# nyu-systems/Grendel-GS

Measured on AMD Instinct MI355X. Metric: training iters/sec (fwd+bwd), higher is better.
Workload: dtype f32

## Files before the change

grendel-gs_amd/csrc/composite.hip:

```cpp
#include "common.h"

namespace {

constexpr float LOG2E = 1.4426950408889634f;
constexpr float ALPHA_MIN = 1.0f / 255.0f;
constexpr float T_STOP = 0.0001f;

__device__ unsigned long long g_walked[2];

#ifdef GSR_STATS
__device__ unsigned long long g_stats[8];
#define GSR_STAT(i, v) do { const unsigned long long sv__ = (unsigned long long)(v); if (lane == 0) atomicAdd(&g_stats[i], sv__); } while (0)
#else
#define GSR_STAT(i, v) do { } while (0)
#endif

struct Entry {
    float x, y;
    float a2, b2, c2;
    float o;
    bool relevant;
};

#ifndef GSR_NO_LOG2O
#define GSR_LOG2O 1
#endif
__device__ __forceinline__ float entry_exponent(const float4 q0, const float4 q1, float dx, float dy) {
#ifdef GSR_LOG2O
    return fmaf(fmaf(q0.z, dx, q0.w * dy), dx, fmaf(q1.x * dy, dy, q1.y));
#else
    return (q0.z * dx + q0.w * dy) * dx + q1.x * dy * dy;
#endif
}
__device__ __forceinline__ float entry_alpha_raw(const float4 q1, float pe) {
#ifdef GSR_LOG2O
    return __builtin_amdgcn_exp2f(pe);
#else
    return q1.y * __builtin_amdgcn_exp2f(pe);
#endif
}
__device__ __forceinline__ bool entry_power_ok(const float4 q1, float pe) {
#ifdef GSR_LOG2O
    return pe <= q1.y;
#else
    return pe <= 0.f;
#endif
}

__device__ __forceinline__ float entry_opacity_term(float o) {
#ifdef GSR_LOG2O
    return __log2f(o);
#else
    return o;
#endif
}

__device__ __forceinline__ Entry load_entry(bool have, uint32_t id, const float2 *__restrict__ means2D,
                                            const float4 *__restrict__ conic_opacity, float qx0, float qy0) {
    Entry e;
    e.x = e.y = e.a2 = e.b2 = e.c2 = e.o = 0.f;
    e.relevant = false;
    if (have) {
        const float2 xy = means2D[id];
        const float4 co = conic_opacity[id];
        e.x = xy.x;
        e.y = xy.y;
        e.a2 = -0.5f * LOG2E * co.x;
        e.b2 = -LOG2E * co.y;
        e.c2 = -0.5f * LOG2E * co.z;
        e.o = entry_opacity_term(co.w);
        e.relevant = gsr_can_touch_box(xy, co, qx0, qy0, qx0 + 7.0f, qy0 + 7.0f);
    }
    return e;
}


typedef float v2f __attribute__((ext_vector_type(2)));
constexpr int PREC = 20;
struct PairRec {
    v2f x, y, a2, b2, c2, o, r, g, b;
};
__device__ __forceinline__ void pair_store(float *__restrict__ slab, int pos, const Entry &e, float r, float g, float b) {
    float *rec = slab + (pos >> 1) * PREC + (pos & 1);
    rec[0] = e.x;  rec[2] = e.y;  rec[4] = e.a2;  rec[6] = e.b2;  rec[8] = e.c2;
    rec[10] = e.o; rec[12] = r;   rec[14] = g;    rec[16] = b;
}
__device__ __forceinline__ PairRec pair_load(const float *__restrict__ slab, int pair) {
    const float4 *q = reinterpret_cast<const float4 *>(slab + pair * PREC);
    const float4 q0 = q[0], q1 = q[1], q2 = q[2], q3 = q[3];
    const float2 q4 = *reinterpret_cast<const float2 *>(q + 4);
    PairRec p;
    p.x = v2f{q0.x, q0.y};  p.y = v2f{q0.z, q0.w};  p.a2 = v2f{q1.x, q1.y};  p.b2 = v2f{q1.z, q1.w};
    p.c2 = v2f{q2.x, q2.y}; p.o = v2f{q2.z, q2.w};  p.r = v2f{q3.x, q3.y};   p.g = v2f{q3.z, q3.w};
    p.b = v2f{q4.x, q4.y};
    return p;
}
__device__ __forceinline__ v2f pair_exponent(const PairRec &p, float pxf, float pyf) {
    const v2f dx = p.x - pxf, dy = p.y - pyf;
    return __builtin_elementwise_fma(__builtin_elementwise_fma(p.a2, dx, p.b2 * dy), dx,
                                     __builtin_elementwise_fma(p.c2 * dy, dy, p.o));
}

__device__ __forceinline__ int composite_tile_of_block(const int2 *__restrict__ ranges, int gx, int tiles) {
    const int2 hull = ranges[tiles];
    const int gy = tiles / gx;
    if (hull.x < 0 || hull.y > gy || hull.x >= hull.y) return gsr_xcd_span_of_block(blockIdx.x, tiles);
    return gsr_xcd_span_of_block_band(blockIdx.x, tiles, hull.x * gx, (hull.y - hull.x) * gx);
}

struct RawEntry {
    float2 xy;
    float4 co;
    float r, g, b;
};
__device__ __forceinline__ RawEntry load_raw(bool have, uint32_t id, const float2 *__restrict__ means2D,
                                             const float4 *__restrict__ conic_opacity, const float *__restrict__ rgb) {
    RawEntry e;
    e.xy = make_float2(0.f, 0.f);
    e.co = make_float4(0.f, 0.f, 0.f, 0.f);
    e.r = e.g = e.b = 0.f;
    if (have) {
        e.xy = means2D[id];
        e.co = conic_opacity[id];
        e.r = rgb[3 * (size_t)id];
        e.g = rgb[3 * (size_t)id + 1];
        e.b = rgb[3 * (size_t)id + 2];
    }
    return e;
}

#ifndef GSR_SEG_LEN
#define GSR_SEG_LEN 256
#endif
#ifndef GSR_SEG_MAXJ
#define GSR_SEG_MAXJ 16
#endif
constexpr int SEG_LEN = GSR_SEG_LEN;
constexpr int SEG_MAXJ = GSR_SEG_MAXJ;
static_assert(SEG_LEN % 64 == 0 && (SEG_LEN & (SEG_LEN - 1)) == 0 && SEG_MAXJ <= 31,
              "segment geometry: K8 finds boundaries with c & (SEG_LEN - 1), so SEG_LEN is a power of two");
constexpr int SEG_WORKERS = 1024;
constexpr int SEG_SLOT_FLOATS = 7 * 256;
struct SegWs {
    uint32_t *hdr;
    uint32_t *queue;
    int32_t *seg_slot;
    float *ckpt;
    uint32_t cap;
};
__host__ __device__ inline size_t seg_ws_bytes(int tiles, uint32_t cap) {
    return 64 + sizeof(uint32_t) * (size_t)cap + sizeof(int32_t) * (size_t)tiles * SEG_MAXJ + sizeof(float) * SEG_SLOT_FLOATS * (size_t)cap;
}
inline SegWs seg_ws_of(void *ws, int tiles, uint32_t cap) {
    SegWs w{};
    if (!ws) return w;
    char *b = reinterpret_cast<char *>(ws);
    w.hdr = reinterpret_cast<uint32_t *>(b);
    w.queue = reinterpret_cast<uint32_t *>(b + 64);
    w.seg_slot = reinterpret_cast<int32_t *>(b + 64 + sizeof(uint32_t) * (size_t)cap);
    w.ckpt = reinterpret_cast<float *>(b + 64 + sizeof(uint32_t) * (size_t)cap + sizeof(int32_t) * (size_t)tiles * SEG_MAXJ);
    w.cap = cap;
    return w;
}
constexpr uint32_t SEG_CAP = 8192;

__device__ __forceinline__ int k8_checkpoint(const SegWs &seg, int *s_slot, int tile, int c, int lane,
                                                       int wave, float T, float c0, float c1, float c2) {
    const int j = c / SEG_LEN - 1;
    int slot = 0;
    if (lane == 0) {
        int v = atomicCAS(&s_slot[j], -1, -2);
        if (v == -1) {
            const uint32_t k = atomicAdd(seg.hdr, 1u);
            v = k < seg.cap ? (int)k : -3;
            if (v >= 0) {
                seg.queue[k] = (uint32_t)tile * 32u + (uint32_t)(j + 1);
                seg.seg_slot[(size_t)tile * SEG_MAXJ + j] = v;
            }
            __hip_atomic_store(&s_slot[j], v, __ATOMIC_RELEASE, __HIP_MEMORY_SCOPE_WORKGROUP);
        } else {
            while (v == -2) v = __hip_atomic_load(&s_slot[j], __ATOMIC_ACQUIRE, __HIP_MEMORY_SCOPE_WORKGROUP);
        }
        slot = v;
    }
    slot = __builtin_amdgcn_readfirstlane(slot);
    if (slot >= 0) {
        float *ck = seg.ckpt + (size_t)slot * SEG_SLOT_FLOATS + wave * 64 + lane;
        ck[0] = T;
        ck[256] = c0;
        ck[512] = c1;
        ck[768] = c2;
    }
    return slot;
}

template <bool SEG, bool BAND>
__global__ void __launch_bounds__(256)
composite_forward_kernel(int W, int H, int gx, const int2 *__restrict__ ranges,
                         const uint32_t *__restrict__ point_list, const float2 *__restrict__ means2D,
                         const float4 *__restrict__ conic_opacity, const float *__restrict__ rgb,
                         const uint8_t *__restrict__ compute_locally, const float *__restrict__ bg,
                         float *__restrict__ out_color, float *__restrict__ final_T, int32_t *__restrict__ n_contrib,
                         const SegWs seg, int band_first, int band_tiles, uint4 *__restrict__ zero16,
                         size_t zero16_n) {
    const size_t HW = (size_t)H * W;
    for (size_t i = (size_t)blockIdx.x * 256 + threadIdx.x; i < zero16_n; i += (size_t)gridDim.x * 256)
        zero16[i] = make_uint4(0u, 0u, 0u, 0u);
    int tile;
    bool idle = false;
    if (BAND) {
        if (band_first < 0) {
            const int gy = (H + GSR_BLOCK_Y - 1) / GSR_BLOCK_Y;
            int2 hull = ranges[gx * gy];
            if (hull.x < 0 || hull.y > gy || hull.x >= hull.y) hull = make_int2(0, 0);
            band_first = hull.x * gx;
            band_tiles = min((hull.y - hull.x) * gx, band_tiles);
            idle = (int)blockIdx.x >= band_tiles;
        }
        tile = band_first + (idle ? 0 : gsr_xcd_span_of_block(blockIdx.x, band_tiles));
    } else {
        tile = composite_tile_of_block(ranges, gx, (int)gridDim.x);
    }
    auto clear_outside = [&]() {
        if (!BAND) return;
        const size_t n0 = (size_t)min(H, (band_first / gx) * GSR_BLOCK_Y) * W;
        const size_t p1 = (size_t)min(H, ((band_first + band_tiles) / gx) * GSR_BLOCK_Y) * W;
        const size_t nout = n0 + (HW - p1);
        for (size_t i = (size_t)blockIdx.x * 256 + threadIdx.x; i < nout; i += (size_t)gridDim.x * 256) {
            const size_t q = i < n0 ? i : p1 + (i - n0);
            out_color[q] = 0.f;
            out_color[HW + q] = 0.f;
            out_color[2 * HW + q] = 0.f;
            final_T[q] = 1.f;
            n_contrib[q] = 0;
        }
    };
    if (idle) {
        clear_outside();
        return;
    }
    const int lane = threadIdx.x & 63, wave = threadIdx.x >> 6;
    const int tx = tile % gx, ty = tile / gx;
    const int qx0 = tx * GSR_BLOCK_X + (wave & 1) * 8, qy0 = ty * GSR_BLOCK_Y + (wave >> 1) * 8;
    const int px = qx0 + (lane & 7), py = qy0 + (lane >> 3);
    const bool inside = px < W && py < H;
    const size_t pid = (size_t)py * W + px;

    if (!compute_locally[tile]) {
        if (inside) {
            out_color[pid] = 0.f;
            out_color[HW + pid] = 0.f;
            out_color[2 * HW + pid] = 0.f;
            final_T[pid] = 1.f;
            n_contrib[pid] = 0;
        }
        clear_outside();
        return;
    }
    const int2 range = ranges[tile];
    const int n = range.y - range.x;
    const float pxf = (float)px, pyf = (float)py;

    float T = 1.0f, C0 = 0.f, C1 = 0.f, C2 = 0.f;
    int last = 0;
    bool done = !inside;
    __shared__ __attribute__((aligned(16))) float slab[4][32 * PREC];
    __shared__ int s_walk[2];
    __shared__ int s_slot[SEG_MAXJ];
    if (threadIdx.x < 2) s_walk[threadIdx.x] = 0;
    if (SEG && threadIdx.x < SEG_MAXJ) {
        s_slot[threadIdx.x] = -1;
        if (seg.seg_slot) seg.seg_slot[(size_t)tile * SEG_MAXJ + threadIdx.x] = -1;
    }
    __syncthreads();
    v2f A0 = {0.f, 0.f}, A1 = {0.f, 0.f}, A2 = {0.f, 0.f};
    v2f B0 = {0.f, 0.f}, B1 = {0.f, 0.f}, B2 = {0.f, 0.f};
    int nstored = 0;
    float *wslab = slab[wave];
    int walked = 0;

    for (int c = 0; c < n; c += 64) {
        if (__all(done)) break;
        if (SEG && seg.seg_slot && c > 0 && (c & (SEG_LEN - 1)) == 0 && c <= SEG_LEN * SEG_MAXJ) {
            if (k8_checkpoint(seg, s_slot, tile, c, lane, wave, T, B0.x + B0.y, B1.x + B1.y, B2.x + B2.y) >= 0) {
                B0 = B1 = B2 = v2f{0.f, 0.f};
                nstored = c / SEG_LEN;
            }
        }
        walked = c + 64;
        const bool have = c + lane < n;
        const uint32_t id = have ? point_list[range.x + c + lane] : 0u;
        const Entry e = load_entry(have, id, means2D, conic_opacity, (float)qx0, (float)qy0);
        float r = 0.f, g = 0.f, b = 0.f;
        if (e.relevant) {
            r = rgb[3 * (size_t)id];
            g = rgb[3 * (size_t)id + 1];
            b = rgb[3 * (size_t)id + 2];
        }
        unsigned long long m = __ballot(e.relevant);
        GSR_STAT(0, __popcll(__ballot(have)));
        GSR_STAT(1, __popcll(m));
        const int nrel = __popcll(m);
        if (e.relevant) pair_store(wslab, __popcll(m & ((1ull << lane) - 1ull)), e, r, g, b);
        {
            const int pad = (-nrel) & 3, slot = nrel + lane / 9;
            if (lane < 9 * pad) wslab[(slot >> 1) * PREC + 2 * (lane % 9) + (slot & 1)] = 0.f;
        }
        for (int p0 = 0; p0 < nrel; p0 += 4) {
            float al[4];
            bool ok[4];
            int kk[4];
            v2f cr[2], cg[2], cb[2];
#pragma unroll
            for (int h = 0; h < 2; h++) {
                const PairRec pr = pair_load(wslab, (p0 >> 1) + h);
                const v2f pe = pair_exponent(pr, pxf, pyf);
                cr[h] = pr.r;
                cg[h] = pr.g;
                cb[h] = pr.b;
#pragma unroll
                for (int u = 0; u < 2; u++) {
                    const bool live = m != 0;
                    kk[2 * h + u] = live ? __builtin_ctzll(m) : 0;
                    m &= m - 1;
                    const float pe1 = u ? pe.y : pe.x, lo = u ? pr.o.y : pr.o.x;
                    al[2 * h + u] = fminf(0.99f, __builtin_amdgcn_exp2f(pe1));
                    ok[2 * h + u] = live && pe1 <= lo && al[2 * h + u] >= ALPHA_MIN;
                }
            }
            float wv[4];
#pragma unroll
            for (int u = 0; u < 4; u++) {
                const bool take = !done && ok[u];
                const float w0 = al[u] * T;
                const float test_T = T - w0;
                const bool stop = take && __float_as_int(test_T) < __float_as_int(T_STOP);
                done = done || stop;
                const bool blend = take && !stop;
                wv[u] = blend ? w0 : 0.f;
                T = blend ? test_T : T;
                last = blend ? c + kk[u] + 1 : last;
            }
#pragma unroll
            for (int h = 0; h < 2; h++) {
                const v2f w2 = {wv[2 * h], wv[2 * h + 1]};
                A0 = __builtin_elementwise_fma(cr[h], w2, A0);
                A1 = __builtin_elementwise_fma(cg[h], w2, A1);
                A2 = __builtin_elementwise_fma(cb[h], w2, A2);
                if (SEG) {
                    B0 = __builtin_elementwise_fma(cr[h], w2, B0);
                    B1 = __builtin_elementwise_fma(cg[h], w2, B1);
                    B2 = __builtin_elementwise_fma(cb[h], w2, B2);
                }
            }
            if (__all(done)) break;
        }
    }
    if (lane == 0) {
        atomicMax(&s_walk[0], walked < n ? walked : n);
        if (atomicAdd(&s_walk[1], 1) == 3) atomicAdd(&g_walked[0], (unsigned long long)s_walk[0]);
    }
    C0 = A0.x + A0.y;
    C1 = A1.x + A1.y;
    C2 = A2.x + A2.y;
    if (SEG && nstored > 0) {
        float r0 = B0.x + B0.y, r1 = B1.x + B1.y, r2 = B2.x + B2.y;
        for (int j = nstored - 1; j >= 0; j--) {
            float *ck = seg.ckpt + (size_t)s_slot[j] * SEG_SLOT_FLOATS + wave * 64 + lane;
            ck[1024] = r0;
            ck[1280] = r1;
            ck[1536] = r2;
            r0 += ck[256];
            r1 += ck[512];
            r2 += ck[768];
        }
    }
    if (inside) {
        out_color[pid] = C0 + T * bg[0];
        out_color[HW + pid] = C1 + T * bg[1];
        out_color[2 * HW + pid] = C2 + T * bg[2];
        final_T[pid] = T;
        n_contrib[pid] = last;
    }
    clear_outside();
}

typedef float f32x4 __attribute__((ext_vector_type(4)));

constexpr int MB = 8;
constexpr int MSTR = 66;

__device__ __forceinline__ void
composite_backward_segment(const int tile, const int sidx, int W, int H, int gx, const int2 *__restrict__ ranges,
                           const uint32_t *__restrict__ point_list, const float2 *__restrict__ means2D,
                           const float4 *__restrict__ conic_opacity, const float *__restrict__ rgb,
                           const uint8_t *__restrict__ compute_locally, const float *__restrict__ bg,
                           const float *__restrict__ final_T, const int32_t *__restrict__ n_contrib,
                           const float *__restrict__ dL_dpixels, double *__restrict__ dL_record,
                           const SegWs &seg, uint8_t *__restrict__ touched) {
    if (!compute_locally[tile]) return;
    const int lane = threadIdx.x & 63, wave = threadIdx.x >> 6;
    const int tx = tile % gx, ty = tile / gx;
    const int qx0 = tx * GSR_BLOCK_X + (wave & 1) * 8, qy0 = ty * GSR_BLOCK_Y + (wave >> 1) * 8;
    const int px = qx0 + (lane & 7), py = qy0 + (lane >> 3);
    const bool inside = px < W && py < H;
    const size_t pid = (size_t)py * W + px;
    const size_t HW = (size_t)H * W;
    const int2 range = ranges[tile];
    const float pxf = (float)px, pyf = (float)py;

    const int c_lo = sidx * SEG_LEN;
    int end_slot = -1;
    if (seg.seg_slot && sidx < SEG_MAXJ) end_slot = seg.seg_slot[(size_t)tile * SEG_MAXJ + sidx];
    const int c_hi = end_slot >= 0 ? c_lo + SEG_LEN : 0x7fffffff;
    const float T_final = inside ? final_T[pid] : 0.f;
    const int last = inside ? n_contrib[pid] : 0;
    float g0 = 0.f, g1 = 0.f, g2 = 0.f;
    if (inside) {
        g0 = dL_dpixels[pid];
        g1 = dL_dpixels[HW + pid];
        g2 = dL_dpixels[2 * HW + pid];
    }
    const float tb = T_final * (bg[0] * g0 + bg[1] * g1 + bg[2] * g2);
    const float ddelx_dx = 0.5f * W, ddely_dy = 0.5f * H;

    __shared__ float2 smat[4][MB * MSTR];
    __shared__ float sacc[4][64 * 9];
    __shared__ __attribute__((aligned(16))) float slab[4][32 * PREC];
    __shared__ float fslab[64 * 7];
    __shared__ float sout[64 * 10];
    __shared__ int s_wmax[4];
    int wmax = min(last, c_hi);
#pragma unroll
    for (int d = 32; d >= 1; d >>= 1) wmax = max(wmax, __shfl_xor(wmax, d, 64));
    if (wmax <= c_lo) wmax = 0;
    if (lane == 0) s_wmax[wave] = wmax;
    for (int i = threadIdx.x; i < 4 * 64 * 9; i += 256) (&sacc[0][0])[i] = 0.f;
    __syncthreads();
    const int bmax = max(max(s_wmax[0], s_wmax[1]), max(s_wmax[2], s_wmax[3]));
    if (bmax == 0) return;
    if (threadIdx.x == 0) atomicAdd(&g_walked[1], (unsigned long long)(bmax - c_lo));
    int wbest = 0;
#pragma unroll
    for (int w = 1; w < 4; w++)
        if (s_wmax[w] > s_wmax[wbest]) wbest = w;

    const int kq = lane >> 4, j = lane & 15;
    float Bop[16];
    {
        const bool isg = j >= 6 && j < 9;
        const float xa = (j == 0 || j == 2 || j == 5) ? 1.f : 0.f, xb1 = (j == 1 || j == 4) ? 1.f : 0.f, xc = j == 3 ? 1.f : 0.f;
        const float ya = (j == 0 || j == 1 || j == 3) ? 1.f : 0.f, yb1 = (j == 2 || j == 4) ? 1.f : 0.f, yc = j == 5 ? 1.f : 0.f;
        const float xl = (float)((wave & 1) * 8 + kq);
        float X[2];
#pragma unroll
        for (int h = 0; h < 2; h++) {
            const float x = xl + 4.f * h;
            X[h] = fmaf(x, fmaf(xc, x, xb1), xa);
        }
        const int gx0 = qx0 + kq;
        const int cx0 = min(gx0, W - 1), cx1 = min(gx0 + 4, W - 1);
        const float *gb = dL_dpixels + (size_t)(isg ? j - 6 : 0) * HW;
        float G[16];
#pragma unroll
        for (int t = 0; t < 16; t++) G[t] = 0.f;
        if (isg) {
#pragma unroll
            for (int t = 0; t < 16; t++) G[t] = gb[(size_t)min(qy0 + (t >> 1), H - 1) * W + ((t & 1) ? cx1 : cx0)];
        }
#pragma unroll
        for (int t = 0; t < 16; t++) {
            const float y = (float)((wave >> 1) * 8 + (t >> 1));
            const float Y = fmaf(y, fmaf(yc, y, yb1), ya);
            const bool inb = ((t & 1) ? gx0 + 4 : gx0) < W && qy0 + (t >> 1) < H;
            Bop[t] = isg ? (inb ? G[t] : 0.f) : X[t & 1] * Y;
        }
    }
    const float *arow = reinterpret_cast<const float *>(&smat[wave][(j & 7) * MSTR + kq]) + (j >> 3);
    const bool my_cols = kq < 2 ? j < 6 : (j >= 6 && j < 9);
    float *wslab = slab[wave];

    float T = T_final;
    float rho = 0.f;
    if (end_slot >= 0 && last > c_hi) {
        const float *ck = seg.ckpt + (size_t)end_slot * SEG_SLOT_FLOATS + wave * 64 + lane;
        T = ck[0];
        rho = (ck[1024] * g0 + ck[1280] * g1 + ck[1536] * g2) * __builtin_amdgcn_rcpf(T);
    }

    const int c0 = ((bmax - 1) / 64) * 64;
    uint32_t id_cur = (c0 + lane < wmax) ? point_list[range.x + c0 + lane] : 0u;
    uint32_t id_nxt = (c0 >= c_lo + 64 && c0 - 64 + lane < wmax) ? point_list[range.x + c0 - 64 + lane] : 0u;
    RawEntry raw = load_raw(c0 + lane < wmax, id_cur, means2D, conic_opacity, rgb);

    for (int c = c0; c >= c_lo; c -= 64) {
        float *acc_tab = sacc[wave];
        const bool have_nxt = c >= c_lo + 64 && c - 64 + lane < wmax;
        const RawEntry raw_nxt = load_raw(have_nxt, id_nxt, means2D, conic_opacity, rgb);
        const uint32_t id_nxt2 = (c >= c_lo + 128 && c - 128 + lane < wmax) ? point_list[range.x + c - 128 + lane] : 0u;
        if (c < wmax) {
            const bool have = c + lane < wmax;
            Entry e;
            e.x = raw.xy.x;
            e.y = raw.xy.y;
            e.a2 = -0.5f * LOG2E * raw.co.x;
            e.b2 = -LOG2E * raw.co.y;
            e.c2 = -0.5f * LOG2E * raw.co.z;
            e.o = entry_opacity_term(raw.co.w);
            e.relevant = have && gsr_can_touch_box(raw.xy, raw.co, (float)qx0, (float)qy0, (float)qx0 + 7.0f, (float)qy0 + 7.0f);
            unsigned long long m = __ballot(e.relevant);
            GSR_STAT(0, __popcll(__ballot(have)));
            GSR_STAT(1, __popcll(m));
            GSR_STAT(6, 1);
            if (e.relevant) pair_store(wslab, __popcll((m >> lane) >> 1), e, raw.r, raw.g, raw.b);
            if (wave == wbest) {
                float *fe = &fslab[7 * lane];
                fe[0] = e.x;  fe[1] = e.y;  fe[2] = e.a2;  fe[3] = e.b2;  fe[4] = e.c2;
                fe[5] = __uint_as_float(id_cur);
                fe[6] = raw.co.w;
            }
            unsigned long long sk = 0ull;
            auto contract_batch = [&](int filled) {
                __builtin_amdgcn_wave_barrier();
                f32x4 acc = {0.f, 0.f, 0.f, 0.f}, acc1 = {0.f, 0.f, 0.f, 0.f};
#pragma unroll
                for (int t = 0; t < 16; t += 2) {
                    acc = __builtin_amdgcn_mfma_f32_16x16x4f32(arow[8 * t], Bop[t], acc, 0, 0, 0);
                    acc1 = __builtin_amdgcn_mfma_f32_16x16x4f32(arow[8 * t + 8], Bop[t + 1], acc1, 0, 0, 0);
                }
                acc += acc1;
                const uint32_t sk4 = (kq & 1) ? (uint32_t)(sk >> 32) : (uint32_t)sk;
#pragma unroll
                for (int r4 = 0; r4 < 4; r4++) {
                    const int slot = 4 * (kq & 1) + r4;
                    if (slot < filled && my_cols) acc_tab[(int)((sk4 >> (8 * r4)) & 0xffu) * 9 + j] = acc[r4];
                }
                GSR_STAT(5, 1);
                __builtin_amdgcn_wave_barrier();
                sk = 0ull;
            };
            int s = 0;
            for (int pi = 0; m; pi++) {
                const int ka = 63 - __builtin_clzll(m);
                m &= ~(1ull << ka);
                const bool two = m != 0ull;
                const int kb = two ? 63 - __builtin_clzll(m) : ka;
                m &= ~(1ull << kb);
                const PairRec pr = pair_load(wslab, pi);
                const v2f pe = pair_exponent(pr, pxf, pyf);
                const float aar = __builtin_amdgcn_exp2f(pe.x), bar = __builtin_amdgcn_exp2f(pe.y);
                const float aal = fminf(0.99f, aar), bal = fminf(0.99f, bar);
                const bool atake = (c + ka + 1 <= last) && pe.x <= pr.o.x && aal >= ALPHA_MIN;
                const bool btake = two && (c + kb + 1 <= last) && pe.y <= pr.o.y && bal >= ALPHA_MIN;
                const v2f cg = __builtin_elementwise_fma(pr.b, v2f{g2, g2}, __builtin_elementwise_fma(pr.g, v2f{g1, g1}, pr.r * g0));
                GSR_STAT(2, two ? 2 : 1);
                GSR_STAT(3, (__builtin_amdgcn_ballot_w64(atake) != 0ull) + (__builtin_amdgcn_ballot_w64(btake) != 0ull));
                GSR_STAT(4, __popcll(__builtin_amdgcn_ballot_w64(atake)) + __popcll(__builtin_amdgcn_ballot_w64(btake)));
                const v2f qa = {atake ? aar : 0.f, atake ? aal : 0.f};
                const v2f qb = {btake ? bar : 0.f, btake ? bal : 0.f};
                const v2f inv = {__builtin_amdgcn_rcpf(1.f - qa.y), __builtin_amdgcn_rcpf(1.f - qb.y)};
                const v2f tbi = inv * tb;
                {
                    const float Tn = T * inv.x;
                    const float dot = cg.x - rho;
                    const float da = fmaf(dot, Tn, -tbi.x);
                    const v2f qw = qa * v2f{da, Tn};
                    smat[wave][s * MSTR + lane] = make_float2(qw.x, qw.y);
                    rho = fmaf(qa.y, dot, rho);
                    T = Tn;
                }
                sk |= (unsigned long long)ka << (8 * s);
                s++;
                if (two) {
                    const float Tn = T * inv.y;
                    const float dot = cg.y - rho;
                    const float da = fmaf(dot, Tn, -tbi.y);
                    const v2f qw = qb * v2f{da, Tn};
                    smat[wave][s * MSTR + lane] = make_float2(qw.x, qw.y);
                    rho = fmaf(qb.y, dot, rho);
                    T = Tn;
                    sk |= (unsigned long long)kb << (8 * s);
                    s++;
                }
                if (s == MB) {
                    contract_batch(MB);
                    s = 0;
                }
            }
            if (s > 0) contract_batch(s);
        }
        __syncthreads();
        if (wave == ((c >> 6) & 3)) {
            const float tx0 = (float)(tx * GSR_BLOCK_X), ty0 = (float)(ty * GSR_BLOCK_Y);
            const int e9 = 9 * lane;
            float Sv[9];
#pragma unroll
            for (int v = 0; v < 9; v++) Sv[v] = (sacc[0][e9 + v] + sacc[1][e9 + v]) + (sacc[2][e9 + v] + sacc[3][e9 + v]);
            const float *fe = &fslab[7 * lane];
            const float ex = fe[0] - tx0, ey = fe[1] - ty0;
            const float cA = fe[2] * (-2.0f / LOG2E), cB = fe[3] * (-1.0f / LOG2E), cC = fe[4] * (-2.0f / LOG2E);
            const float A0 = Sv[0], Ax = Sv[1], Ay = Sv[2];
            const float Mx = fmaf(ex, A0, -Ax), My = fmaf(ey, A0, -Ay);
            float o[9];
            o[0] = -(cA * Mx + cB * My) * ddelx_dx;
            o[1] = -(cB * Mx + cC * My) * ddely_dy;
            o[2] = Sv[6];
            o[3] = Sv[7];
            o[4] = Sv[8];
            o[5] = -0.5f * (fmaf(fmaf(ex, A0, -2.f * Ax), ex, Sv[3]));
            o[6] = -(fmaf(ex, My, -ey * Ax) + Sv[4]);
            o[7] = -0.5f * (fmaf(fmaf(ey, A0, -2.f * Ay), ey, Sv[5]));
            o[8] = A0 == 0.f ? 0.f : A0 / fe[6];
            const bool live = c + lane < bmax;
            float *so = &sout[10 * lane];
#pragma unroll
            for (int v = 0; v < 9; v++) so[v] = live ? o[v] : 0.f;
            so[9] = fe[5];
        }
        __syncthreads();
#pragma unroll
        for (int r = 0; r < 3; r++) {
            const int idx = threadIdx.x + 256 * r;
            const int e = idx / 9, col = idx - 9 * e;
            if (idx < 576) {
                const float val = sout[10 * e + col];
#ifndef GSR_ABL_NOATOMIC
                if (val != 0.f) {
                    const uint32_t id = __float_as_uint(sout[10 * e + 9]);
                    atomicAdd(dL_record + 9 * (size_t)id + col, (double)val);
                    if (touched) touched[id] = 1;
                }
#else
                asm volatile("" ::"v"(val));
#endif
            }
        }
#pragma unroll
        for (int i = 0; i < 9; i++) acc_tab[64 * i + lane] = 0.f;
        raw = raw_nxt;
        id_cur = id_nxt;
        id_nxt = id_nxt2;
    }
}

// ... 159 lines not shown
```

grendel-gs_amd/csrc/loss.hip:

```cpp
#include "common.h"

namespace {

__constant__ const float WIN[11] = {1.0283801239e-03f, 7.5987582095e-03f, 3.6000773311e-02f, 1.0936068743e-01f,
                                    2.1300552785e-01f, 2.6601171494e-01f, 2.1300552785e-01f, 1.0936068743e-01f,
                                    3.6000773311e-02f, 7.5987582095e-03f, 1.0283801239e-03f};
constexpr int LT = 512;
constexpr int VO = 1024 / LT;
constexpr int TW = 32, TH = 32;
constexpr int HW = TW + 10, HH = TH + 10;
constexpr int HSTR = TW + 8;
constexpr int TS = TW;
constexpr float SSIM_C1 = 0.01f * 0.01f;
constexpr float SSIM_C2 = 0.03f * 0.03f;

__device__ __forceinline__ float block_sum(float v, float *smem) {
    const int lane = threadIdx.x & 63, wave = threadIdx.x >> 6;
#pragma unroll
    for (int d = 32; d >= 1; d >>= 1) v += __shfl_xor(v, d, 64);
    if (lane == 0) smem[wave] = v;
    __syncthreads();
    float r = 0.f;
    for (int w = 0; w < LT / 64; w++) r += smem[w];
    __syncthreads();
    return r;
}

typedef float v2f __attribute__((ext_vector_type(2)));

__device__ __forceinline__ int loss_tile(int gxT, int gyT, int &c, int &ox, int &oy, int nwg) {
    const int lin = gsr_xcd_span_of_block(blockIdx.x, nwg);
    c = lin / (gxT * gyT);
    const int rem = lin - c * (gxT * gyT);
    const int by = rem / gxT;
    ox = (rem - by * gxT) * TW;
    oy = by * TH;
    return lin;
}
__device__ __forceinline__ bool loss_band(const int *__restrict__ band, int rows_cap, int W, int gxT, int &rows, int &gyT,
                                          int &nwg, long long &row_off) {
    nwg = gridDim.x;
    row_off = 0;
    if (!band) return true;
    const int channels = nwg / (gxT * gyT);
    const int y0 = band[0], y1 = band[1];
    rows = max(0, min(y1 - y0, rows_cap));
    gyT = (rows + TH - 1) / TH;
    nwg = channels * gxT * gyT;
    row_off = (long long)y0 * W;
    return (int)blockIdx.x < nwg;
}
constexpr int HV = (TW + 16) / 4;
static_assert(HH * HV <= LT, "one halo vector per thread");

__device__ __forceinline__ float expo_apply(const float *e, float x0, float x1, float x2) {
    return fmaf(e[0], x0, fmaf(e[1], x1, fmaf(e[2], x2, e[3])));
}

template <bool VEC, bool EXPO>
__global__ void __launch_bounds__(LT)
l1_ssim_forward_kernel(int rows, int W, int gxT, int gyT, const float *__restrict__ image, long long img_cstride,
                       const uint8_t *__restrict__ gt, float *__restrict__ partials, float *__restrict__ M1,
                       float *__restrict__ M2, float *__restrict__ M3, const int *__restrict__ band,
                       const float *__restrict__ expo) {
    __shared__ v2f sXY[HH][HW + 1];
    __shared__ v2f hAB[HH][HSTR];
    __shared__ v2f hCD[HH][HSTR];
    __shared__ float hE[HH][HSTR];
    __shared__ float red[LT / 64];
    int c, ox, oy, nwg;
    long long row_off;
    const int rows_cap = rows;
    if (!loss_band(band, rows_cap, W, gxT, rows, gyT, nwg, row_off)) {
        if (threadIdx.x < 2) partials[2 * (size_t)blockIdx.x + threadIdx.x] = 0.f;
        return;
    }
    const int tile_id = loss_tile(gxT, gyT, c, ox, oy, nwg);
    const int tid = threadIdx.x;
    const float *img_c = image + (long long)c * img_cstride + row_off;
    const uint8_t *gt_c = gt + (size_t)c * rows_cap * W;
    float e[4] = {0.f, 0.f, 0.f, 0.f};
    if (EXPO) {
#pragma unroll
        for (int i = 0; i < 4; i++) e[i] = expo[4 * c + i];
    }
    const float *img_0 = image + row_off;
    if (VEC) {
        if (tid < HH * HV) {
            const int ly = tid / HV, q = tid - ly * HV;
            const int gy = oy + ly - 5, gx0 = ox - 8 + 4 * q;
            float4 x = make_float4(0.f, 0.f, 0.f, 0.f);
            uchar4 y = make_uchar4(0, 0, 0, 0);
            if (gy >= 0 && gy < rows && gx0 >= 0 && gx0 < W) {
                if (EXPO) {
                    const float *p = img_0 + (size_t)gy * W + gx0;
                    const float4 x0 = *reinterpret_cast<const float4 *>(p);
                    const float4 x1 = *reinterpret_cast<const float4 *>(p + img_cstride);
                    const float4 x2 = *reinterpret_cast<const float4 *>(p + 2 * img_cstride);
                    x = make_float4(expo_apply(e, x0.x, x1.x, x2.x), expo_apply(e, x0.y, x1.y, x2.y),
                                    expo_apply(e, x0.z, x1.z, x2.z), expo_apply(e, x0.w, x1.w, x2.w));
                } else {
                    x = *reinterpret_cast<const float4 *>(img_c + (size_t)gy * W + gx0);
                }
                y = *reinterpret_cast<const uchar4 *>(gt_c + (size_t)gy * W + gx0);
            }
            const float xs[4] = {x.x, x.y, x.z, x.w};
            const float ys[4] = {(float)y.x, (float)y.y, (float)y.z, (float)y.w};
#pragma unroll
            for (int i = 0; i < 4; i++) {
                const int lx = 4 * q - 3 + i;
                if (lx >= 0 && lx < HW) sXY[ly][lx] = v2f{xs[i], ys[i] * (1.0f / 255.0f)};
            }
        }
    } else {
        for (int idx = tid; idx < HH * HW; idx += LT) {
            const int ly = idx / HW, lx = idx % HW;
            const int gy = oy + ly - 5, gx = ox + lx - 5;
            v2f v = {0.f, 0.f};
            if (gy >= 0 && gy < rows && gx >= 0 && gx < W) {
                if (EXPO) {
                    const float *p = img_0 + (size_t)gy * W + gx;
                    v.x = expo_apply(e, p[0], p[img_cstride], p[2 * img_cstride]);
                } else {
                    v.x = img_c[(size_t)gy * W + gx];
                }
                v.y = (float)gt_c[(size_t)gy * W + gx] * (1.0f / 255.0f);
            }
            sXY[ly][lx] = v;
        }
    }
    __syncthreads();
    for (int task = tid; task < HH * (TW / 4); task += LT) {
        const int r = task / (TW / 4), cx0 = (task % (TW / 4)) * 4;
        v2f xy[14], sq[14];
        float pr[14];
#pragma unroll
        for (int i = 0; i < 14; i++) {
            xy[i] = sXY[r][cx0 + i];
            sq[i] = xy[i] * xy[i];
            pr[i] = xy[i].x * xy[i].y;
        }
#pragma unroll
        for (int o = 0; o < 4; o++) {
            v2f a = {0.f, 0.f}, b = {0.f, 0.f};
            float e = 0.f;
#pragma unroll
            for (int k = 0; k < 11; k++) {
                const float w = WIN[k];
                a += xy[o + k] * w;
                b += sq[o + k] * w;
                e += pr[o + k] * w;
            }
            hAB[r][cx0 + o] = a;
            hCD[r][cx0 + o] = b;
            hE[r][cx0 + o] = e;
        }
    }
    __syncthreads();
    const int tx = tid % TW, ty0 = (tid / TW) * VO;
    v2f vab[VO], vcd[VO];
    float ve[VO];
    {
        v2f p[10 + VO], q[10 + VO];
        float t[10 + VO];
#pragma unroll
        for (int i = 0; i < 10 + VO; i++) {
            p[i] = hAB[ty0 + i][tx];
            q[i] = hCD[ty0 + i][tx];
            t[i] = hE[ty0 + i][tx];
        }
#pragma unroll
        for (int o = 0; o < VO; o++) {
            v2f a = {0.f, 0.f}, b = {0.f, 0.f};
            float e = 0.f;
#pragma unroll
            for (int k = 0; k < 11; k++) {
                const float w = WIN[k];
                a += p[o + k] * w;
                b += q[o + k] * w;
                e += t[o + k] * w;
            }
            vab[o] = a;
            vcd[o] = b;
            ve[o] = e;
        }
    }
    const int gx = ox + tx;
    float l1 = 0.f, ssim_sum = 0.f;
#pragma unroll
    for (int o = 0; o < VO; o++) {
        const int ty = ty0 + o, gy = oy + ty;
        if (gy < rows && gx < W) {
            const float mu1 = vab[o].x, mu2 = vab[o].y, e11 = vcd[o].x, e22 = vcd[o].y, e12 = ve[o];
            const v2f cxy = sXY[ty + 5][tx + 5];
            const float x = cxy.x, y = cxy.y;
            const float mu1_sq = mu1 * mu1, mu2_sq = mu2 * mu2, mu12 = mu1 * mu2;
            const float s1 = e11 - mu1_sq, s2 = e22 - mu2_sq, s12 = e12 - mu12;
            const float A = 2.f * mu12 + SSIM_C1, B = 2.f * s12 + SSIM_C2;
            const float Cd = mu1_sq + mu2_sq + SSIM_C1, Dd = s1 + s2 + SSIM_C2;
            const float inv_d = __builtin_amdgcn_rcpf(Dd);
            const float inv = __builtin_amdgcn_rcpf(Cd) * inv_d;
            const float ssim = A * B * inv;
            ssim_sum += ssim;
            l1 += fabsf(x - y);
            if (M1) {
                const size_t off = ((size_t)c * rows_cap + gy) * W + gx;
                M1[off] = 2.f * mu2 * (B - A) * inv - ssim * 2.f * mu1 * (Dd - Cd) * inv;
                M2[off] = -ssim * inv_d;
                M3[off] = 2.f * A * inv;
            }
        }
    }
    const float sl1 = block_sum(l1, red);
    const float sss = block_sum(ssim_sum, red);
    if (tid == 0) {
        partials[2 * (size_t)tile_id] = sl1;
        partials[2 * (size_t)tile_id + 1] = sss;
    }
}

template <bool VEC>
__global__ void __launch_bounds__(LT)
l1_ssim_backward_kernel(int rows, int W, int gxT, int gyT, const float *__restrict__ image, long long img_cstride,
                        const uint8_t *__restrict__ gt, const float *__restrict__ M1, const float *__restrict__ M2,
                        const float *__restrict__ M3, const float *__restrict__ grad_l1_sum,
                        const float *__restrict__ grad_ssim_sum, float scale_l1, float scale_ssim,
                        float *__restrict__ grad_image, long long grad_cstride, const int *__restrict__ band) {
    __shared__ float sM[3][HH][HW + 1];
    __shared__ float hor[3][HH][HSTR];
    int c, ox, oy, nwg;
    long long row_off;
    const int rows_cap = rows;
    if (!loss_band(band, rows_cap, W, gxT, rows, gyT, nwg, row_off)) return;
    loss_tile(gxT, gyT, c, ox, oy, nwg);
    const int tid = threadIdx.x;
    const size_t cbase = (size_t)c * rows_cap * W;
    if (VEC) {
        if (tid < HH * HV) {
            const int ly = tid / HV, q = tid - ly * HV;
            const int gy = oy + ly - 5, gx0 = ox - 8 + 4 * q;
            float4 a = make_float4(0.f, 0.f, 0.f, 0.f), b = a, d = a;
            if (gy >= 0 && gy < rows && gx0 >= 0 && gx0 < W) {
                const size_t o = cbase + (size_t)gy * W + gx0;
                a = *reinterpret_cast<const float4 *>(M1 + o);
                b = *reinterpret_cast<const float4 *>(M2 + o);
                d = *reinterpret_cast<const float4 *>(M3 + o);
            }
            const float as[4] = {a.x, a.y, a.z, a.w}, bs[4] = {b.x, b.y, b.z, b.w}, ds[4] = {d.x, d.y, d.z, d.w};
#pragma unroll
            for (int i = 0; i < 4; i++) {
                const int lx = 4 * q - 3 + i;
                if (lx >= 0 && lx < HW) {
                    sM[0][ly][lx] = as[i];
                    sM[1][ly][lx] = bs[i];
                    sM[2][ly][lx] = ds[i];
                }
            }
        }
    } else {
        for (int idx = tid; idx < HH * HW; idx += LT) {
            const int ly = idx / HW, lx = idx % HW;
            const int gy = oy + ly - 5, gx = ox + lx - 5;
            float a = 0.f, b = 0.f, d = 0.f;
            if (gy >= 0 && gy < rows && gx >= 0 && gx < W) {
                const size_t o = cbase + (size_t)gy * W + gx;
                a = M1[o];
                b = M2[o];
                d = M3[o];
            }
            sM[0][ly][lx] = a;
            sM[1][ly][lx] = b;
            sM[2][ly][lx] = d;
        }
    }
    __syncthreads();
    for (int task = tid; task < HH * (TW / 4); task += LT) {
        const int r = task / (TW / 4), cx0 = (task % (TW / 4)) * 4;
#pragma unroll
        for (int m = 0; m < 3; m++) {
            float v[14];
#pragma unroll
            for (int i = 0; i < 14; i++) v[i] = sM[m][r][cx0 + i];
#pragma unroll
            for (int o = 0; o < 4; o++) {
                float a = 0.f;
#pragma unroll
                for (int k = 0; k < 11; k++) a += WIN[k] * v[o + k];
                hor[m][r][cx0 + o] = a;
            }
        }
    }
    __syncthreads();
    const int tx = tid % TW, ty0 = (tid / TW) * VO;
    float cv[3][VO];
#pragma unroll
    for (int m = 0; m < 3; m++) {
        float v[10 + VO];
#pragma unroll
        for (int i = 0; i < 10 + VO; i++) v[i] = hor[m][ty0 + i][tx];
#pragma unroll
        for (int o = 0; o < VO; o++) {
            float a = 0.f;
#pragma unroll
            for (int k = 0; k < 11; k++) a += WIN[k] * v[o + k];
            cv[m][o] = a;
        }
    }
    const int gx = ox + tx;
    if (gx >= W) return;
    const float gl1 = grad_l1_sum[0] * scale_l1, gss = grad_ssim_sum[0] * scale_ssim;
#pragma unroll
    for (int o = 0; o < VO; o++) {
        const int gy = oy + ty0 + o;
        if (gy >= rows) break;
        const float x = image[(long long)c * img_cstride + row_off + (size_t)gy * W + gx];
        const float y = (float)gt[cbase + (size_t)gy * W + gx] * (1.0f / 255.0f);
        const float d = x - y;
        const float sgn = (d > 0.f ? 1.f : 0.f) - (d < 0.f ? 1.f : 0.f);
        grad_image[(long long)c * grad_cstride + row_off + (size_t)gy * W + gx] =
            gl1 * sgn + gss * (cv[0][o] + 2.f * x * cv[1][o] + y * cv[2][o]);
    }
}

__global__ void __launch_bounds__(256) l1_ssim_finalize_kernel(int nb, const float *__restrict__ partials, float c_l1,
                                                                float c_ssim, float bias, float inv_n,
                                                                float *__restrict__ out) {
    __shared__ double red[2][4];
    double a = 0.0, b = 0.0;
    const float2 *p2 = reinterpret_cast<const float2 *>(partials);
    for (int i0 = threadIdx.x; i0 < nb; i0 += 256 * 8) {
        float2 v[8];
#pragma unroll
        for (int u = 0; u < 8; u++) v[u] = p2[min(i0 + 256 * u, nb - 1)];
#pragma unroll
        for (int u = 0; u < 8; u++)
            if (i0 + 256 * u < nb) {
                a += (double)v[u].x;
                b += (double)v[u].y;
            }
    }
#pragma unroll
    for (int d = 32; d >= 1; d >>= 1) {
        a += __shfl_xor(a, d, 64);
        b += __shfl_xor(b, d, 64);
    }
    if ((threadIdx.x & 63) == 0) {
        red[0][threadIdx.x >> 6] = a;
        red[1][threadIdx.x >> 6] = b;
    }
    __syncthreads();
    if (threadIdx.x == 0) {
        const float s1 = (float)(red[0][0] + red[0][1] + red[0][2] + red[0][3]);
        const float s2 = (float)(red[1][0] + red[1][1] + red[1][2] + red[1][3]);
        out[0] = c_l1 * s1 + c_ssim * s2 + bias;
        out[1] = s1 * inv_n;
        out[2] = s2 * inv_n;
    }
}

template <bool VEC>
__global__ void __launch_bounds__(LT)
l1_ssim_backward_exposure_kernel(int rows, int W, int gxT, int gyT, const float *__restrict__ image, long long img_cstride,
                                 const uint8_t *__restrict__ gt, const float *__restrict__ M1,
                                 const float *__restrict__ M2, const float *__restrict__ M3,
                                 const float *__restrict__ grad_l1_sum, const float *__restrict__ grad_ssim_sum,
                                 float scale_l1, float scale_ssim, float *__restrict__ grad_image, long long grad_cstride,
                                 const int *__restrict__ band, const float *__restrict__ expo,
                                 float *__restrict__ expo_partials) {
    __shared__ float sM[3][HH][HW + 1];
    __shared__ float hor[3][HH][HSTR];
    __shared__ float red[12][LT / 64];
    int c0, ox, oy, nwg;
    long long row_off;
    const int rows_cap = rows;
    if (!loss_band(band, rows_cap, W, gxT, rows, gyT, nwg, row_off)) {
        if (threadIdx.x < 12) expo_partials[12 * (size_t)blockIdx.x + threadIdx.x] = 0.f;
        return;
    }
    const int tile_id = loss_tile(gxT, gyT, c0, ox, oy, nwg);
    const int tid = threadIdx.x, lane = tid & 63, wave = tid >> 6;
    const int tx = tid % TW, ty0 = (tid / TW) * VO;
    const int gx = ox + tx;
    const float gl1 = grad_l1_sum[0] * scale_l1, gss = grad_ssim_sum[0] * scale_ssim;
    float xin[3][VO], gout[3][VO];
    bool ok[VO];
#pragma unroll
    for (int o = 0; o < VO; o++) {
        const int gy = oy + ty0 + o;
        ok[o] = gx < W && gy < rows;
#pragma unroll
        for (int k = 0; k < 3; k++) {
            xin[k][o] = ok[o] ? image[(long long)k * img_cstride + row_off + (size_t)gy * W + gx] : 0.f;
            gout[k][o] = 0.f;
        }
    }
#pragma unroll 1
    for (int c = 0; c < 3; c++) {
        const size_t cbase = (size_t)c * rows_cap * W;
        if (VEC) {
            if (tid < HH * HV) {
                const int ly = tid / HV, q = tid - ly * HV;
                const int gy = oy + ly - 5, gx0 = ox - 8 + 4 * q;
                float4 a = make_float4(0.f, 0.f, 0.f, 0.f), b = a, d = a;
                if (gy >= 0 && gy < rows && gx0 >= 0 && gx0 < W) {
                    const size_t o = cbase + (size_t)gy * W + gx0;
                    a = *reinterpret_cast<const float4 *>(M1 + o);
                    b = *reinterpret_cast<const float4 *>(M2 + o);
                    d = *reinterpret_cast<const float4 *>(M3 + o);
                }
                const float as[4] = {a.x, a.y, a.z, a.w}, bs[4] = {b.x, b.y, b.z, b.w}, ds[4] = {d.x, d.y, d.z, d.w};
#pragma unroll
                for (int i = 0; i < 4; i++) {
                    const int lx = 4 * q - 3 + i;
                    if (lx >= 0 && lx < HW) {
                        sM[0][ly][lx] = as[i];
                        sM[1][ly][lx] = bs[i];
                        sM[2][ly][lx] = ds[i];
                    }
                }
            }
        } else {
            for (int idx = tid; idx < HH * HW; idx += LT) {
                const int ly = idx / HW, lx = idx % HW;
                const int gy = oy + ly - 5, gxh = ox + lx - 5;
                float a = 0.f, b = 0.f, d = 0.f;
                if (gy >= 0 && gy < rows && gxh >= 0 && gxh < W) {
                    const size_t o = cbase + (size_t)gy * W + gxh;
                    a = M1[o];
                    b = M2[o];
                    d = M3[o];
                }
                sM[0][ly][lx] = a;
                sM[1][ly][lx] = b;
                sM[2][ly][lx] = d;
            }
        }
        __syncthreads();
        for (int task = tid; task < HH * (TW / 4); task += LT) {
            const int r = task / (TW / 4), cx0 = (task % (TW / 4)) * 4;
#pragma unroll
            for (int m = 0; m < 3; m++) {
                float v[14];
#pragma unroll
                for (int i = 0; i < 14; i++) v[i] = sM[m][r][cx0 + i];
#pragma unroll
                for (int o = 0; o < 4; o++) {
                    float a = 0.f;
#pragma unroll
                    for (int k = 0; k < 11; k++) a = fmaf(WIN[k], v[o + k], a);
                    hor[m][r][cx0 + o] = a;
                }
            }
        }
        __syncthreads();
        float cv[3][VO];
#pragma unroll
        for (int m = 0; m < 3; m++) {
            float v[10 + VO];
#pragma unroll
            for (int i = 0; i < 10 + VO; i++) v[i] = hor[m][ty0 + i][tx];
#pragma unroll
            for (int o = 0; o < VO; o++) {
                float a = 0.f;
#pragma unroll
                for (int k = 0; k < 11; k++) a = fmaf(WIN[k], v[o + k], a);
                cv[m][o] = a;
            }
        }
        float e[4];
#pragma unroll
        for (int i = 0; i < 4; i++) e[i] = expo[4 * c + i];
        float s[4] = {0.f, 0.f, 0.f, 0.f};
#pragma unroll
        for (int o = 0; o < VO; o++) {
            float gp = 0.f;
            if (ok[o]) {
                const int gy = oy + ty0 + o;
                const float x = expo_apply(e, xin[0][o], xin[1][o], xin[2][o]);
                const float y = (float)gt[cbase + (size_t)gy * W + gx] * (1.0f / 255.0f);
                const float d = x - y;
                const float sgn = (d > 0.f ? 1.f : 0.f) - (d < 0.f ? 1.f : 0.f);
                const float inner = __fadd_rn(__fadd_rn(cv[0][o], __fmul_rn(__fmul_rn(2.f, x), cv[1][o])),
                                              __fmul_rn(y, cv[2][o]));
                gp = __fadd_rn(__fmul_rn(gl1, sgn), __fmul_rn(gss, inner));
            }
#pragma unroll
            for (int k = 0; k < 3; k++) {
                gout[k][o] = fmaf(e[k], gp, gout[k][o]);
                s[k] = fmaf(gp, xin[k][o], s[k]);
            }
            s[3] += gp;
        }
#pragma unroll
        for (int j = 0; j < 4; j++) {
            float v = s[j];
#pragma unroll
            for (int d = 32; d >= 1; d >>= 1) v += __shfl_xor(v, d, 64);
            if (lane == 0) red[4 * c + j][wave] = v;
        }
    }
    __syncthreads();
    if (tid < 12) {
        float r = 0.f;
        for (int w = 0; w < LT / 64; w++) r += red[tid][w];
        expo_partials[12 * (size_t)tile_id + tid] = r;
    }
#pragma unroll
    for (int o = 0; o < VO; o++) {
        if (!ok[o]) continue;
        const int gy = oy + ty0 + o;
#pragma unroll
        for (int k = 0; k < 3; k++)
            grad_image[(long long)k * grad_cstride + row_off + (size_t)gy * W + gx] = gout[k][o];
    }
}

constexpr int EXPO_GROUPS = 21;
// ... 168 lines not shown
```

Measured before the change: 801.2.

## Store contributor index in pair slab, set occupancy bounds, merge loss reductions

The forward composite kernel now writes each relevant Gaussian's contributor index into the spare slot of its pair record and reads it back, so the per-element ctz/mask walk is no longer needed. Padding records get a sentinel opacity value. Launch bounds now request a minimum occupancy per template variant. In the loss forward kernel, empty asm barriers are meant to steer register allocation, and the two block reductions are merged so they share one barrier. Tighter occupancy bounds may cause register spills.

```diff
diff --git a/grendel-gs_amd/csrc/composite.hip b/grendel-gs_amd/csrc/composite.hip
--- a/grendel-gs_amd/csrc/composite.hip
+++ b/grendel-gs_amd/csrc/composite.hip
@@ -85,6 +85,26 @@
     rec[0] = e.x;  rec[2] = e.y;  rec[4] = e.a2;  rec[6] = e.b2;  rec[8] = e.c2;
     rec[10] = e.o; rec[12] = r;   rec[14] = g;    rec[16] = b;
 }
+__device__ __forceinline__ void pair_store_last(float *__restrict__ slab, int pos, int last) {
+    slab[(pos >> 1) * PREC + 18 + (pos & 1)] = __int_as_float(last);
+}
+__device__ __forceinline__ PairRec pair_load_last(const float *__restrict__ slab, int pair, int &la, int &lb) {
+    const float4 *q = reinterpret_cast<const float4 *>(slab + pair * PREC);
+    const float4 q0 = q[0], q1 = q[1], q2 = q[2], q3 = q[3], q4 = q[4];
+    PairRec p;
+    p.x = v2f{q0.x, q0.y};  p.y = v2f{q0.z, q0.w};  p.a2 = v2f{q1.x, q1.y};  p.b2 = v2f{q1.z, q1.w};
+    p.c2 = v2f{q2.x, q2.y}; p.o = v2f{q2.z, q2.w};  p.r = v2f{q3.x, q3.y};   p.g = v2f{q3.z, q3.w};
+    p.b = v2f{q4.x, q4.y};
+    la = __float_as_int(q4.z);
+    lb = __float_as_int(q4.w);
+    asm("" : "+v"(la), "+v"(lb));
+    return p;
+}
+#ifdef GSR_LOG2O
+#define GSR_PAD_O (-__builtin_inff())
+#else
+#define GSR_PAD_O 0.f
+#endif
 __device__ __forceinline__ PairRec pair_load(const float *__restrict__ slab, int pair) {
     const float4 *q = reinterpret_cast<const float4 *>(slab + pair * PREC);
     const float4 q0 = q[0], q1 = q[1], q2 = q[2], q3 = q[3];
@@ -195,7 +215,7 @@
 }
 
 template <bool SEG, bool BAND>
-__global__ void __launch_bounds__(256)
+__global__ void __launch_bounds__(256, SEG ? 6 : (BAND ? 7 : 8))
 composite_forward_kernel(int W, int H, int gx, const int2 *__restrict__ ranges,
                          const uint32_t *__restrict__ point_list, const float2 *__restrict__ means2D,
                          const float4 *__restrict__ conic_opacity, const float *__restrict__ rgb,
@@ -301,11 +321,23 @@
         GSR_STAT(0, __popcll(__ballot(have)));
         GSR_STAT(1, __popcll(m));
         const int nrel = __popcll(m);
+#ifdef GSR_ABL_K8_MASKWALK
         if (e.relevant) pair_store(wslab, __popcll(m & ((1ull << lane) - 1ull)), e, r, g, b);
         {
             const int pad = (-nrel) & 3, slot = nrel + lane / 9;
             if (lane < 9 * pad) wslab[(slot >> 1) * PREC + 2 * (lane % 9) + (slot & 1)] = 0.f;
         }
+#else
+        if (e.relevant) {
+            const int pos = __popcll(m & ((1ull << lane) - 1ull));
+            pair_store(wslab, pos, e, r, g, b);
+            pair_store_last(wslab, pos, c + lane + 1);
+        }
+        {
+            const int pad = (-nrel) & 3, slot = nrel + lane / 10, f = lane % 10;
+            if (lane < 10 * pad) wslab[(slot >> 1) * PREC + 2 * f + (slot & 1)] = f == 5 ? GSR_PAD_O : 0.f;
+        }
+#endif
         for (int p0 = 0; p0 < nrel; p0 += 4) {
             float al[4];
             bool ok[4];
@@ -313,16 +345,24 @@
             v2f cr[2], cg[2], cb[2];
 #pragma unroll
             for (int h = 0; h < 2; h++) {
+#ifdef GSR_ABL_K8_MASKWALK
                 const PairRec pr = pair_load(wslab, (p0 >> 1) + h);
+#else
+                const PairRec pr = pair_load_last(wslab, (p0 >> 1) + h, kk[2 * h], kk[2 * h + 1]);
+#endif
                 const v2f pe = pair_exponent(pr, pxf, pyf);
                 cr[h] = pr.r;
                 cg[h] = pr.g;
                 cb[h] = pr.b;
 #pragma unroll
                 for (int u = 0; u < 2; u++) {
+#ifdef GSR_ABL_K8_MASKWALK
                     const bool live = m != 0;
-                    kk[2 * h + u] = live ? __builtin_ctzll(m) : 0;
+                    kk[2 * h + u] = c + (live ? __builtin_ctzll(m) : 0) + 1;
                     m &= m - 1;
+#else
+                    const bool live = true;
+#endif
                     const float pe1 = u ? pe.y : pe.x, lo = u ? pr.o.y : pr.o.x;
                     al[2 * h + u] = fminf(0.99f, __builtin_amdgcn_exp2f(pe1));
                     ok[2 * h + u] = live && pe1 <= lo && al[2 * h + u] >= ALPHA_MIN;
@@ -331,15 +371,15 @@
             float wv[4];
 #pragma unroll
             for (int u = 0; u < 4; u++) {
-                const bool take = !done && ok[u];
                 const float w0 = al[u] * T;
                 const float test_T = T - w0;
+                const bool take = !done && ok[u];
                 const bool stop = take && __float_as_int(test_T) < __float_as_int(T_STOP);
                 done = done || stop;
                 const bool blend = take && !stop;
                 wv[u] = blend ? w0 : 0.f;
                 T = blend ? test_T : T;
-                last = blend ? c + kk[u] + 1 : last;
+                last = blend ? kk[u] : last;
             }
 #pragma unroll
             for (int h = 0; h < 2; h++) {
diff --git a/grendel-gs_amd/csrc/loss.hip b/grendel-gs_amd/csrc/loss.hip
--- a/grendel-gs_amd/csrc/loss.hip
+++ b/grendel-gs_amd/csrc/loss.hip
@@ -68,6 +68,9 @@
     __shared__ v2f hCD[HH][HSTR];
     __shared__ float hE[HH][HSTR];
     __shared__ float red[LT / 64];
+#ifndef GSR_ABL_LOSS_TWO_REDUCTIONS
+    __shared__ float red2[LT / 64];
+#endif
     int c, ox, oy, nwg;
     long long row_off;
     const int rows_cap = rows;
@@ -139,6 +142,9 @@
             xy[i] = sXY[r][cx0 + i];
             sq[i] = xy[i] * xy[i];
             pr[i] = xy[i].x * xy[i].y;
+#ifndef GSR_ABL_LOSS_FWD_OUTPUT_PAIRS
+            asm("" : "+v"(pr[i]));
+#endif
         }
 #pragma unroll
         for (int o = 0; o < 4; o++) {
@@ -168,6 +174,9 @@
             p[i] = hAB[ty0 + i][tx];
             q[i] = hCD[ty0 + i][tx];
             t[i] = hE[ty0 + i][tx];
+#ifndef GSR_ABL_LOSS_FWD_OUTPUT_PAIRS
+            asm("" : "+v"(t[i]));
+#endif
         }
 #pragma unroll
         for (int o = 0; o < VO; o++) {
@@ -211,8 +220,24 @@
             }
         }
     }
+#ifdef GSR_ABL_LOSS_TWO_REDUCTIONS
     const float sl1 = block_sum(l1, red);
     const float sss = block_sum(ssim_sum, red);
+#else
+    float sl1 = l1, sss = ssim_sum;
+#pragma unroll
+    for (int d = 32; d >= 1; d >>= 1) sl1 += __shfl_xor(sl1, d, 64);
+#pragma unroll
+    for (int d = 32; d >= 1; d >>= 1) sss += __shfl_xor(sss, d, 64);
+    if ((tid & 63) == 0) {
+        red[tid >> 6] = sl1;
+        red2[tid >> 6] = sss;
+    }
+    __syncthreads();
+    sl1 = sss = 0.f;
+    for (int w = 0; w < LT / 64; w++) sl1 += red[w];
+    for (int w = 0; w < LT / 64; w++) sss += red2[w];
+#endif
     if (tid == 0) {
         partials[2 * (size_t)tile_id] = sl1;
         partials[2 * (size_t)tile_id + 1] = sss;
```

Result: faster. 815.9, median of 6 (+1.8%).
